# valeoai/NAF

Hardware: AMD Instinct MI355X
Metric: upsampled Mpixels/sec (NAF forward) (higher is better)
Workload: dtype bf16; 1 GPU; G1: 1x3x1024x1024 guidance, 1x768x64x64 features -> 1024x1024, window 7, per GPU; per_gpu_batch=1, global_batch=1, parallelism=batch-shard x1, scope=whole forward (conv stem + RoPE/pool + attention), weights=random-init NAF() defaults (dim 256, 4 heads), streams=2

## Files before the change

naf_amd/csrc/stem_conv1x1.hip:

```cpp
#include <type_traits>

#include "naf_common.h"

struct StemConv1Params {
    const bf16_t* x;
    bf16_t* y;
    const bf16_t* w;
    const float* bias;
    const float* gamma;
    const float* beta;
    const double* stats_in;
    double* stats_out;
    int32_t B, H, W;
    int32_t groups_per_image;
    int32_t groups_per_block;
    float eps;
    int64_t xs[3], ys[3];
    const void* img;
    const float* w0;
    const float* b0;
    int64_t ibs;
    int32_t is[4];
    bf16_t* kout;
    const float* tab_y;
    const float* tab_x;
    int64_t kst[3];
    int32_t cw;
    int32_t ncell;
    int32_t cells_per_block;
};

namespace {
constexpr int C1 = 128, WROW = C1 + 8, OROW1 = C1 + 8;
#ifndef NAF_C1X1_NW
#define NAF_C1X1_NW 4
#endif
#ifndef NAF_C1_ABL
#define NAF_C1_ABL 0
#endif
constexpr int NW1 = NAF_C1X1_NW;
typedef float f32x16_t __attribute__((ext_vector_type(16)));
constexpr float kLog2e = 1.4426950408889634f;
}

#ifdef NAF_C1_TIMING
__device__ unsigned long long g_c1_tim[4096 * 8];
#define C1_T(i) do { const unsigned long long now_ = __builtin_amdgcn_s_memtime(); tacc[i] += now_ - tlast; tlast = now_; } while (0)
#else
#define C1_T(i) do { } while (0)
#endif

template <bool IMG, typename T, bool DENSE, bool PLAIN = false, bool POOL = false>
__global__ __launch_bounds__(NW1 * 64, (NW1 <= 4 ? 2 : 1)) void stem_conv1x1_kernel(const StemConv1Params p) {
    static_assert(!(IMG && PLAIN), "the recomputed-conv0 input exists for the forward layer only");
    static_assert(!POOL || (DENSE && !IMG && !PLAIN), "key pooling: dense forward layer reading its input from memory");
#ifdef NAF_C1_TIMING
    unsigned long long tacc[8] = {0, 0, 0, 0, 0, 0, 0, 0}, tlast = __builtin_amdgcn_s_memtime();
#endif
    extern __shared__ __attribute__((aligned(16))) unsigned char smem[];
    bf16_t* wl = reinterpret_cast<bf16_t*>(smem);
    bf16_t* ot = wl + C1 * WROW;
    float* cvec = reinterpret_cast<float*>(ot + NW1 * 32 * OROW1);

    const int tid = threadIdx.x, lane = tid & 63;
    const int wave = __builtin_amdgcn_readfirstlane(tid >> 6);
    const int n32 = lane & 31, half = lane >> 5;
    const int b = blockIdx.y;

    const int gbase = POOL ? blockIdx.x * p.cells_per_block : blockIdx.x * p.groups_per_block;
    const int ngroups = POOL ? min(p.ncell, gbase + p.cells_per_block) : min(p.groups_per_image, gbase + p.groups_per_block);
    const int gstride = NW1;
    const int npx = p.H * p.W;
    bf16_t* otw = ot + wave * 32 * OROW1;

    const int chk = lane & 15, psub = lane >> 4;
    const bool xdense = DENSE || p.xs[1] == (int64_t)p.W * p.xs[2], ydense = DENSE || p.ys[1] == (int64_t)p.W * p.ys[2];
    const bf16_t* xbase = p.x + b * p.xs[0] + chk * 8;
    const uint32_t lane_x = (uint32_t)(psub * (int)p.xs[2] + chk * 8) * 2u, lane_y = (uint32_t)(psub * (int)p.ys[2] + chk * 8) * 2u;
    const int nfull = npx >> 5;
    auto pool_group_off = [&](int cell, int gi, const int64_t (&st)[3]) __attribute__((always_inline)) {
        const int cc = cell < ngroups ? cell : ngroups - 1;
        const int cy = cc / p.cw, cx = cc - cy * p.cw;
        return (int64_t)(cy * 16 + 2 * gi) * st[1] + (int64_t)cx * 16 * st[2];
    };
    auto load_group = [&](int g, u32x4_t (&raw)[8], int gi = 0) __attribute__((always_inline)) {
        if constexpr (POOL) {
            const char* xg = reinterpret_cast<const char*>(p.x + b * p.xs[0] + pool_group_off(g, gi, p.xs));
            uint32_t lx = lane_x;
            asm volatile("" : "+v"(lx));
#pragma unroll
            for (int it = 0; it < 8; ++it)
                raw[it] = *reinterpret_cast<const u32x4_t*>(xg + (uint32_t)(lx + (uint32_t)(((it >> 2) * (int)p.xs[1] + (it & 3) * 4 * (int)p.xs[2]) * 2)));
            return;
        }
        const int gc = g < ngroups ? g : ngroups - 1;
        if (DENSE || (xdense && gc < nfull)) {
            const char* xg = reinterpret_cast<const char*>(p.x + b * p.xs[0] + (int64_t)gc * 32 * p.xs[2]);
            uint32_t lx = lane_x;
            asm volatile("" : "+v"(lx));
#pragma unroll
            for (int it = 0; it < 8; ++it) raw[it] = *reinterpret_cast<const u32x4_t*>(xg + (uint32_t)(lx + (uint32_t)(it * 8 * (int)p.xs[2])));
            return;
        }
        if constexpr (!DENSE) {
#pragma unroll
        for (int it = 0; it < 8; ++it) {
            const int n = min(gc * 32 + it * 4 + psub, npx - 1);
            int64_t off;
            if (xdense) {
                off = (int64_t)n * p.xs[2];
            } else {
                const int yy = n / p.W, xx = n - yy * p.W;
                off = (int64_t)yy * p.xs[1] + (int64_t)xx * p.xs[2];
            }
            raw[it] = *reinterpret_cast<const u32x4_t*>(xbase + off);
        }
        }
    };
    constexpr int WCH = C1 * (C1 / 8), WIT = (WCH + NW1 * 64 - 1) / (NW1 * 64);
    u32x4_t wst[WIT];
#pragma unroll
    for (int i = 0; i < WIT; ++i) {
        const int ci = min(tid + i * NW1 * 64, WCH - 1);
        wst[i] = *reinterpret_cast<const u32x4_t*>(p.w + (ci >> 4) * C1 + (ci & 15) * 8);
    }
    u32x4_t raw[8];
    if constexpr (!IMG) load_group(gbase + wave, raw);
#pragma unroll
    for (int i = 0; i < WIT; ++i) {
        const int ci = tid + i * NW1 * 64;
        if (WCH % (NW1 * 64) == 0 || ci < WCH) *reinterpret_cast<u32x4_t*>(wl + (ci >> 4) * WROW + (ci & 15) * 8) = wst[i];
    }
    if (tid < C1) {
        const int c = tid, g = c >> 4;
        if constexpr (PLAIN) {
            cvec[c] = p.bias ? p.bias[c] : 0.f;
        } else {
            const double n = (double)p.H * (double)p.W * 16.0;
            double s1, s2;
            naf_gn_sums(p.stats_in, p.B, b, g, s1, s2);
            const double mean = s1 / n;
            double var = s2 / n - mean * mean;
            var = var > 0.0 ? var : 0.0;
            const float rstd = (float)(1.0 / sqrt(var + (double)p.eps));
            const float gmm = p.gamma[c];
            cvec[c] = p.bias[c];
            cvec[C1 + c] = gmm * rstd * kLog2e;
            cvec[2 * C1 + c] = (p.beta[c] - (float)mean * gmm * rstd) * kLog2e;
            if constexpr (IMG) cvec[3 * C1 + c] = p.b0[c];
        }
    }
    __syncthreads();

    float ga[8], gb[8];
#pragma unroll
    for (int e = 0; e < 8; ++e) {
        ga[e] = cvec[C1 + chk * 8 + e];
        gb[e] = cvec[2 * C1 + chk * 8 + e];
    }

    f32x2_t s1p[8], s2p[8];
#pragma unroll
    for (int g = 0; g < 8; ++g) s1p[g] = s2p[g] = f32x2_t{0.f, 0.f};

    float w0r[4][2];
    const T* ib = nullptr;
    if constexpr (IMG) {
        ib = reinterpret_cast<const T*>(p.img) + (int64_t)b * p.ibs;
#pragma unroll
        for (int m = 0; m < 4; ++m)
#pragma unroll
            for (int ks = 0; ks < 2; ++ks) {
                const int k = 2 * ks + half;
                w0r[m][ks] = (k < 3) ? p.w0[(32 * m + n32) * 3 + k] : 0.f;
            }
    }
    auto load_taps = [&](int g, float (&sv)[2]) __attribute__((always_inline)) {
        const int gc = g < ngroups ? g : ngroups - 1;
        const int n = min(gc * 32 + n32, npx - 1);
        const int yy = n / p.W, xx = n - yy * p.W;
        const int o = yy * p.is[2] + xx * p.is[3];
        sv[0] = (float)ib[o + half * p.is[1]];
        sv[1] = (float)ib[o + 2 * p.is[1]];
    };

    float sv[2] = {0.f, 0.f};
    int g = gbase + wave;
    int gi = 0;
    f32x4_t pacc[8];
    float ptab[16];
    bf16x8_t pax;
    const int pG = lane >> 4, pli = lane & 15;
    if constexpr (POOL) {
#pragma unroll
        for (int j = 0; j < 8; ++j) pacc[j] = f32x4_t{0.f, 0.f, 0.f, 0.f};
#pragma unroll
        for (int i = 0; i < 16; ++i) ptab[i] = 0.f;
#pragma unroll
        for (int i = 0; i < 8; ++i) pax[i] = (bf16_t)((8 * (pG & 1) + i == pli) ? 1.0f : 0.0f);
    }
    if constexpr (IMG) load_taps(g, sv);
    if constexpr (IMG) asm volatile("; conv1x1 first group landed" ::"v"(sv[0]), "v"(sv[1]));
    else asm volatile("; conv1x1 first group landed" ::"v"(raw[0]), "v"(raw[1]), "v"(raw[2]), "v"(raw[3]), "v"(raw[4]), "v"(raw[5]), "v"(raw[6]), "v"(raw[7]));
    C1_T(0);
    for (; g < ngroups; g += (POOL ? 0 : gstride)) {
        const int n0 = g * 32;
#ifdef NAF_C1_TIMING
        if constexpr (!IMG) {
            asm volatile("s_waitcnt vmcnt(8)" ::: "memory");
            C1_T(1);
        }
#endif
        const float* cv = cvec;

        f32x16_t acc[4];
#pragma unroll
        for (int m = 0; m < 4; ++m)
#pragma unroll
            for (int j = 0; j < 4; ++j) {
                const f32x4_t bj = *reinterpret_cast<const f32x4_t*>(cv + 32 * m + 8 * j + 4 * half);
#pragma unroll
                for (int i = 0; i < 4; ++i) acc[m][j * 4 + i] = bj[i];
            }
        if constexpr (IMG) {
#pragma unroll
            for (int mp = 0; mp < 2; ++mp) {
                f32x16_t a0[2];
#pragma unroll
                for (int q = 0; q < 2; ++q) {
#pragma unroll
                    for (int r = 0; r < 16; ++r) a0[q][r] = 0.f;
#pragma unroll
                    for (int ks = 0; ks < 2; ++ks) a0[q] = __builtin_amdgcn_mfma_f32_32x32x2f32(w0r[2 * mp + q][ks], sv[ks], a0[q], 0, 0, 0);
                }
#pragma unroll
                for (int q = 0; q < 2; ++q) {
                    const int m = 2 * mp + q;
#pragma unroll
                    for (int j = 0; j < 4; ++j) {
                        const int c0 = 32 * m + 8 * j + 4 * half;
                        const f32x4_t bj = *reinterpret_cast<const f32x4_t*>(cv + 3 * C1 + c0);
                        const f32x4_t gaj = *reinterpret_cast<const f32x4_t*>(cv + C1 + c0);
                        const f32x4_t gbj = *reinterpret_cast<const f32x4_t*>(cv + 2 * C1 + c0);
                        bf16x4_t o;
#pragma unroll
                        for (int e = 0; e < 2; ++e) {
                            const f32x2_t v = f32x2_t{a0[q][j * 4 + 2 * e], a0[q][j * 4 + 2 * e + 1]} + f32x2_t{bj[2 * e], bj[2 * e + 1]};
                            bf16x2_t xb;
                            xb[0] = (bf16_t)v[0];
                            xb[1] = (bf16_t)v[1];
                            const f32x2_t x = {(float)xb[0], (float)xb[1]};
                            const f32x2_t y = x * f32x2_t{gaj[2 * e], gaj[2 * e + 1]} + f32x2_t{gbj[2 * e], gbj[2 * e + 1]};
                            const f32x2_t u = f32x2_t{__builtin_amdgcn_exp2f(-y[0]), __builtin_amdgcn_exp2f(-y[1])} * kLog2e + kLog2e;
                            const f32x2_t r = y * f32x2_t{__builtin_amdgcn_rcpf(u[0]), __builtin_amdgcn_rcpf(u[1])};
                            o[2 * e] = (bf16_t)r[0];
                            o[2 * e + 1] = (bf16_t)r[1];
                        }
                        *reinterpret_cast<bf16x4_t*>(otw + n32 * OROW1 + c0) = o;
                    }
                }
            }
        } else {
#pragma unroll
        for (int it = 0; it < 8; ++it) {
            if constexpr (PLAIN || (NAF_C1_ABL & 1)) {
                *reinterpret_cast<u32x4_t*>(otw + (it * 4 + psub) * OROW1 + chk * 8) = raw[it];
                continue;
            }
            bf16x8_t o;
#pragma unroll
            for (int e = 0; e < 4; ++e) {
                const uint32_t w = raw[it][e];
                const f32x2_t x = {__uint_as_float(w << 16), __uint_as_float(w & 0xffff0000u)};
                const f32x2_t y = x * f32x2_t{ga[2 * e], ga[2 * e + 1]} + f32x2_t{gb[2 * e], gb[2 * e + 1]};
                const f32x2_t u = f32x2_t{__builtin_amdgcn_exp2f(-y[0]), __builtin_amdgcn_exp2f(-y[1])} * kLog2e + kLog2e;
                const f32x2_t r = y * f32x2_t{__builtin_amdgcn_rcpf(u[0]), __builtin_amdgcn_rcpf(u[1])};
                o[2 * e] = (bf16_t)r[0];
                o[2 * e + 1] = (bf16_t)r[1];
            }
            *reinterpret_cast<bf16x8_t*>(otw + (it * 4 + psub) * OROW1 + chk * 8) = o;
        }
        }
        C1_T(2);
        __builtin_amdgcn_sched_barrier(0);
        if constexpr (IMG) load_taps(g + gstride, sv);
        else if constexpr (POOL) {
            load_group(gi == 7 ? g + gstride : g, raw, (gi + 1) & 7);
            if (gi == 7) {
                const int cy = g / p.cw, cx = g - cy * p.cw;
                const float* ty = p.tab_y + (int64_t)(cy * 16 + 4 * pG) * 32 + pli;
                const float* tx = p.tab_x + (int64_t)(cx * 16 + 4 * pG) * 32 + pli;
#pragma unroll
                for (int i = 0; i < 4; ++i) {
                    ptab[i] = ty[i * 32];
                    ptab[4 + i] = ty[i * 32 + 16];
                    ptab[8 + i] = tx[i * 32];
                    ptab[12 + i] = tx[i * 32 + 16];
                }
            }
        }
        else if constexpr (!(NAF_C1_ABL & 16)) load_group(g + gstride, raw);
        __builtin_amdgcn_sched_barrier(0);
        {
            bf16x8_t bfr[2], war[2][4];
            auto frag = [&](int ks, int slot) __attribute__((always_inline)) {
                bfr[slot] = *reinterpret_cast<const bf16x8_t*>(otw + n32 * OROW1 + ks * 16 + half * 8);
#pragma unroll
                for (int m = 0; m < 4; ++m) war[slot][m] = *reinterpret_cast<const bf16x8_t*>(wl + (m * 32 + n32) * WROW + ks * 16 + half * 8);
            };
            frag(0, 0);
#pragma unroll
            for (int ks = 0; ks < 8; ++ks) {
                __builtin_amdgcn_sched_barrier(0);
                if (ks + 1 < 8) frag(ks + 1, (ks + 1) & 1);
                __builtin_amdgcn_sched_barrier(0);
#pragma unroll
                for (int m = 0; m < 4; ++m) {
                    if constexpr (!(NAF_C1_ABL & 2)) acc[m] = __builtin_amdgcn_mfma_f32_32x32x16_bf16(war[ks & 1][m], bfr[ks & 1], acc[m], 0, 0, 0);
                    else asm volatile("" ::"v"(war[ks & 1][m]), "v"(bfr[ks & 1]));
                }
            }
            __builtin_amdgcn_sched_barrier(0);
        }
#ifdef NAF_C1_TIMING
        asm volatile("" ::"v"(acc[0]), "v"(acc[1]), "v"(acc[2]), "v"(acc[3]));
        C1_T(3);
#endif
        const bool full = DENSE || g < nfull;
        auto epilogue = [&](auto fullc) __attribute__((always_inline)) {
            constexpr bool FULL = decltype(fullc)::value;
            const float vmask = (FULL || (n0 + n32) < npx) ? 1.0f : 0.0f;
#pragma unroll
            for (int m = 0; m < 4; ++m)
#pragma unroll
                for (int j = 0; j < 4; ++j) {
                    const f32x2_t v0 = f32x2_t{acc[m][j * 4], acc[m][j * 4 + 1]}, v1 = f32x2_t{acc[m][j * 4 + 2], acc[m][j * 4 + 3]};
                    bf16x4_t o;
                    o[0] = (bf16_t)v0[0]; o[1] = (bf16_t)v0[1]; o[2] = (bf16_t)v1[0]; o[3] = (bf16_t)v1[1];
                    const f32x2_t w0 = FULL ? v0 : v0 * vmask, w1 = FULL ? v1 : v1 * vmask;
                    if constexpr (!(NAF_C1_ABL & 4) && !POOL) {
                        s1p[m * 2 + (j >> 1)] += w0 + w1;
                        s2p[m * 2 + (j >> 1)] += w0 * w0 + w1 * w1;
                    }
                    *reinterpret_cast<bf16x4_t*>(otw + n32 * OROW1 + 32 * m + 8 * j + 4 * half) = o;
                }
            C1_T(4);
            bf16_t* yb = p.y + b * p.ys[0];
            if constexpr (POOL) {
                char* yg = reinterpret_cast<char*>(yb + pool_group_off(g, gi, p.ys));
                uint32_t ly = lane_y;
                asm volatile("" : "+v"(ly));
#pragma unroll
                for (int it = 0; it < 8; ++it) {
                    const u32x4_t v = *reinterpret_cast<const u32x4_t*>(otw + (it * 4 + psub) * OROW1 + chk * 8);
                    *reinterpret_cast<u32x4_t*>(yg + (uint32_t)(ly + (uint32_t)(((it >> 2) * (int)p.ys[1] + (it & 3) * 4 * (int)p.ys[2]) * 2))) = v;
                }
                return;
            }
            if (FULL && (DENSE || ydense)) {
                char* yg = reinterpret_cast<char*>(yb + (int64_t)g * 32 * p.ys[2]);
                uint32_t ly = lane_y;
                asm volatile("" : "+v"(ly));
#pragma unroll
                for (int it = 0; it < 8; ++it) {
                    const u32x4_t v = *reinterpret_cast<const u32x4_t*>(otw + (it * 4 + psub) * OROW1 + chk * 8);
                    if constexpr (!(NAF_C1_ABL & 8)) *reinterpret_cast<u32x4_t*>(yg + (int64_t)it * 8 * p.ys[2] + ly) = v;
                    else asm volatile("" ::"v"(v));
                }
                C1_T(5);
                return;
            }
            if constexpr (!(FULL && DENSE)) {
#pragma unroll
            for (int it = 0; it < 8; ++it) {
                const int pp = it * 4 + psub, ch = chk;
                const int n = n0 + pp;
                if (n < npx) {
                    int64_t off;
                    if (ydense) {
                        off = (int64_t)n * p.ys[2];
                    } else {
                        const int yy = n / p.W, xx = n - yy * p.W;
                        off = (int64_t)yy * p.ys[1] + (int64_t)xx * p.ys[2];
                    }
                    const u32x4_t v = *reinterpret_cast<const u32x4_t*>(otw + pp * OROW1 + ch * 8);
                    *reinterpret_cast<u32x4_t*>(yb + off + ch * 8) = v;
                }
            }
            }
        };
        if constexpr (DENSE) {
            epilogue(std::true_type{});
        } else {
            if (full) epilogue(std::true_type{});
            else epilogue(std::false_type{});
        }
        if constexpr (POOL) {
            bf16x8_t pay;
            {
                const bf16_t one = (bf16_t)(((2 * gi + (pG >> 1)) == pli) ? 1.0f : 0.0f);
#pragma unroll
                for (int i = 0; i < 8; ++i) pay[i] = one;
            }
            const bf16_t* tb = otw + (8 * pG + (pli >> 2)) * OROW1 + (pli & 3) * 4;
#pragma unroll
            for (int j = 0; j < 8; ++j) {
                const bf16x4_t lo = __builtin_amdgcn_ds_read_tr16_b64_v4bf16((NAF_LDS bf16x4_t*)(tb + 16 * j));
                const bf16x4_t hi = __builtin_amdgcn_ds_read_tr16_b64_v4bf16((NAF_LDS bf16x4_t*)(tb + 4 * OROW1 + 16 * j));
                const bf16x8_t bt = {lo[0], lo[1], lo[2], lo[3], hi[0], hi[1], hi[2], hi[3]};
                pacc[j] = __builtin_amdgcn_mfma_f32_16x16x32_bf16((j & 1) ? pax : pay, bt, pacc[j], 0, 0, 0);
            }
            if (gi == 7) {
                const int cy = g / p.cw, cx = g - cy * p.cw;
                bf16_t* kc = p.kout + b * p.kst[0] + (int64_t)cy * p.kst[1] + (int64_t)cx * p.kst[2];
#pragma unroll
                for (int hh = 0; hh < 2; ++hh) {
                    float o[4] = {0.f, 0.f, 0.f, 0.f};
#pragma unroll
                    for (int i = 0; i < 4; ++i) {
                        float r1, r2;
                        naf_rope_rotate(pacc[4 * hh][i], pacc[4 * hh + 2][i], ptab[i], ptab[4 + i], r1, r2);
                        o[0] += r1;
                        o[2] += r2;
                        naf_rope_rotate(pacc[4 * hh + 1][i], pacc[4 * hh + 3][i], ptab[8 + i], ptab[12 + i], r1, r2);
                        o[1] += r1;
                        o[3] += r2;
                    }
#pragma unroll
                    for (int q = 0; q < 4; ++q) {
                        o[q] += __shfl_xor(o[q], 16);
                        o[q] += __shfl_xor(o[q], 32);
                    }
                    const float v = pG == 0 ? o[0] : pG == 1 ? o[1] : pG == 2 ? o[2] : o[3];
                    kc[64 * hh + lane] = (bf16_t)(v * (1.0f / 256.0f));
                }
#pragma unroll
                for (int j = 0; j < 8; ++j) pacc[j] = f32x4_t{0.f, 0.f, 0.f, 0.f};
                gi = 0;
                g += gstride;
            } else {
                ++gi;
            }
        }
    }

    if constexpr (IMG) asm volatile("; conv1x1 loop drained" ::"v"(sv[0]), "v"(sv[1]));
    else asm volatile("; conv1x1 loop drained" ::"v"(raw[0]), "v"(raw[1]), "v"(raw[2]), "v"(raw[3]), "v"(raw[4]), "v"(raw[5]), "v"(raw[6]), "v"(raw[7]));
#ifdef NAF_C1_TIMING
    if (lane == 0 && blockIdx.x < 512)
        for (int i = 0; i < 8; ++i) g_c1_tim[(blockIdx.x * NW1 + wave) * 8 + i] = tacc[i];
#endif
    if (p.stats_out) {
        __syncthreads();
        float* red = reinterpret_cast<float*>(ot);
#pragma unroll
        for (int gq = 0; gq < 8; ++gq) {
            float a = s1p[gq][0] + s1p[gq][1], q = s2p[gq][0] + s2p[gq][1];
#pragma unroll
            for (int o = 32; o > 0; o >>= 1) {
                a += __shfl_xor(a, o);
                q += __shfl_xor(q, o);
            }
            if (lane == 0) {
                red[wave * 16 + gq] = a;
                red[wave * 16 + 8 + gq] = q;
            }
        }
        __syncthreads();
        if (tid < 16) {
            float a = 0.f;
#pragma unroll
            for (int wv = 0; wv < NW1; ++wv) a += red[wv * 16 + tid];
            atomicAdd(&naf_gn_slot(p.stats_out, p.B, b, blockIdx.x)[(tid & 7) * 2 + (tid >> 3)], (double)a);
        }
    }
}

int naf_stem_conv1x1_keys_ok(const naf_stem_conv_args* a, const naf_key_pool_args* kp) {
    return a->ksize == 1 && a->first == nullptr && a->stats_in != nullptr && a->stats_out == nullptr && (a->channels == 0 || a->channels == 128) &&
           a->H == 16 * kp->h && a->W == 16 * kp->w && a->x_stride[1] == (int64_t)a->W * a->x_stride[2] &&
           a->y_stride[1] == (int64_t)a->W * a->y_stride[2] && a->x_stride[1] * 2 < 0x7fffffffLL && a->y_stride[1] * 2 < 0x7fffffffLL;
}

int naf_launch_stem_conv1x1(const naf_stem_conv_args* a, hipStream_t s, const naf_key_pool_args* kp) {
    StemConv1Params p;
    p.x = static_cast<const bf16_t*>(a->x);
    p.y = static_cast<bf16_t*>(a->y);
    p.w = static_cast<const bf16_t*>(a->w_packed);
    p.bias = a->bias; p.gamma = a->gn_weight; p.beta = a->gn_bias;
    p.stats_in = a->stats_in; p.stats_out = a->stats_out;
    p.B = a->B; p.H = a->H; p.W = a->W; p.eps = a->eps;
    for (int i = 0; i < 3; ++i) { p.xs[i] = a->x_stride[i]; p.ys[i] = a->y_stride[i]; }
    p.groups_per_image = (int)(((int64_t)a->H * a->W + 31) / 32);
    const size_t lds = (size_t)(C1 * WROW + NW1 * 32 * OROW1) * 2 + 4 * C1 * sizeof(float);
    const int64_t slots = (int64_t)naf_cu_count() * (NW1 <= 4 ? 2 : 1) * NW1;
    const int64_t total = (int64_t)p.groups_per_image * a->B;
    const int64_t gpw = (total + slots - 1) / slots;
    static const int gpw_knob = [] { const char* e = naf_knob("NAF_C1X1_GPW"); return e ? atoi(e) : 0; }();
    const int64_t gpw_eff = gpw_knob > 0 ? gpw_knob : gpw;
    p.groups_per_block = (int32_t)(gpw_eff * NW1);
    int64_t nbx = (p.groups_per_image + p.groups_per_block - 1) / p.groups_per_block;
    if (nbx < 1) nbx = 1;
    if (a->B > 65535) {
        naf_set_error("naf_stem_conv_fwd: batch %d out of range", a->B);
        return NAF_ERR_INVALID;
    }
    p.img = nullptr; p.w0 = nullptr; p.b0 = nullptr; p.ibs = 0;
    for (int i = 0; i < 4; ++i) p.is[i] = 0;
    p.kout = nullptr; p.tab_y = p.tab_x = nullptr; p.cw = p.ncell = p.cells_per_block = 0;
    for (int i = 0; i < 3; ++i) p.kst[i] = 0;
    if (kp != nullptr) {
        if (!naf_stem_conv1x1_keys_ok(a, kp)) {
            naf_set_error("naf_stem_conv_keys_fwd: the 1x1 kernel needs 16 x 16 pixel cells, dense rows, stats_out == NULL and first == NULL");
            return NAF_ERR_UNSUPPORTED;
        }
        p.kout = static_cast<bf16_t*>(kp->k_lr); p.tab_y = kp->tab_y; p.tab_x = kp->tab_x;
        for (int i = 0; i < 3; ++i) p.kst[i] = kp->k_stride[i];
        p.cw = kp->w; p.ncell = kp->h * kp->w;
        const int64_t cpw = ((int64_t)p.ncell * a->B + slots - 1) / slots;
        p.cells_per_block = (int32_t)(cpw * NW1);
        nbx = (p.ncell + p.cells_per_block - 1) / p.cells_per_block;
    }
    int variant = 0;
    if (a->first != nullptr) {
        const naf_stem_conv0_args* f = a->first;
        const int64_t span = 2 * llabs(f->image_stride[1]) + (int64_t)(a->H - 1) * llabs(f->image_stride[2]) +
                             (int64_t)(a->W - 1) * llabs(f->image_stride[3]);
        if (span >= 0x7fffffffLL) {
            naf_set_error("naf_stem_conv_fwd: first: image too large for 32-bit tap offsets (span %lld elements)", (long long)span);
            return NAF_ERR_UNSUPPORTED;
        }
        p.img = f->image; p.w0 = f->weight; p.b0 = f->bias; p.ibs = f->image_stride[0];
        for (int i = 0; i < 4; ++i) p.is[i] = (int32_t)f->image_stride[i];
        variant = f->image_dtype == NAF_BF16 ? 2 : 1;
    }
    const dim3 grid((uint32_t)nbx, (uint32_t)a->B), blk(NW1 * 64);
    if (kp != nullptr) {
        auto kern = stem_conv1x1_kernel<false, float, true, false, true>;
        if (hipFuncSetAttribute(reinterpret_cast<const void*>(kern), hipFuncAttributeMaxDynamicSharedMemorySize, (int)lds) != hipSuccess) {
            naf_set_error("naf_stem_conv_keys_fwd: cannot reserve %zu bytes of LDS", (size_t)lds);
            return NAF_ERR_LAUNCH;
        }
        hipLaunchKernelGGL(kern, grid, blk, lds, s, p);
        return naf_check_launch("stem_conv1x1_kernel<keys>");
    }
#define NAF_LAUNCH_1X1(KERN)                                                                                              \
    do {                                                                                                                  \
        if (hipFuncSetAttribute(reinterpret_cast<const void*>(KERN), hipFuncAttributeMaxDynamicSharedMemorySize, (int)lds) != hipSuccess) { \
            naf_set_error("naf_stem_conv_fwd: cannot reserve %zu bytes of LDS", (size_t)lds);                             \
            return NAF_ERR_LAUNCH;                                                                                        \
        }                                                                                                                 \
        hipLaunchKernelGGL(KERN, grid, blk, lds, s, p);                                                                   \
    } while (0)
    const bool dense = (a->x_stride[1] == (int64_t)a->W * a->x_stride[2] || a->first != nullptr) &&
                       a->y_stride[1] == (int64_t)a->W * a->y_stride[2] && (((int64_t)a->H * a->W) % 32 == 0);
    if (a->stats_in == nullptr) {
        if (dense) NAF_LAUNCH_1X1((stem_conv1x1_kernel<false, float, true, true>));
        else NAF_LAUNCH_1X1((stem_conv1x1_kernel<false, float, false, true>));
    } else if (dense) {
        if (variant == 0) NAF_LAUNCH_1X1((stem_conv1x1_kernel<false, float, true>));
        else if (variant == 1) NAF_LAUNCH_1X1((stem_conv1x1_kernel<true, float, true>));
        else NAF_LAUNCH_1X1((stem_conv1x1_kernel<true, bf16_t, true>));
    } else {
        if (variant == 0) NAF_LAUNCH_1X1((stem_conv1x1_kernel<false, float, false>));
        else if (variant == 1) NAF_LAUNCH_1X1((stem_conv1x1_kernel<true, float, false>));
        else NAF_LAUNCH_1X1((stem_conv1x1_kernel<true, bf16_t, false>));
    }
#undef NAF_LAUNCH_1X1
    return naf_check_launch("stem_conv1x1_kernel");
}
```

Before: 566.8 Mpix/s.

## Keep conv1x1 weights resident in AGPRs and switch to 16x16x32 MFMA

Loads the 128x128 weight matrix once into accumulation registers (AGPRs) per lane, staging it through the per-wave tile region so the dedicated weight LDS area can be dropped. The GEMM moves from 32x32x16 MFMAs with per-step weight fragment LDS reads to 16x16x32 MFMAs using inline asm. The work is split into two 16-pixel halves, so the epilogue and store of one half can interleave with the compute of the next. Pool table loads are moved next to their use, and non-dense inputs are now loaded inside the loop rather than prefetched. This removes LDS weight traffic and shrinks the LDS footprint, at the cost of many AGPRs, hand-placed nops for hazards, and less overlap of the next group's load in the non-dense path.

```diff
diff --git a/naf_amd/csrc/stem_conv1x1.hip b/naf_amd/csrc/stem_conv1x1.hip
--- a/naf_amd/csrc/stem_conv1x1.hip
+++ b/naf_amd/csrc/stem_conv1x1.hip
@@ -31,7 +31,7 @@
 };
 
 namespace {
-constexpr int C1 = 128, WROW = C1 + 8, OROW1 = C1 + 8;
+constexpr int C1 = 128, OROW1 = C1 + 8;
 #ifndef NAF_C1X1_NW
 #define NAF_C1X1_NW 4
 #endif
@@ -58,13 +58,15 @@
     unsigned long long tacc[8] = {0, 0, 0, 0, 0, 0, 0, 0}, tlast = __builtin_amdgcn_s_memtime();
 #endif
     extern __shared__ __attribute__((aligned(16))) unsigned char smem[];
-    bf16_t* wl = reinterpret_cast<bf16_t*>(smem);
-    bf16_t* ot = wl + C1 * WROW;
+    bf16_t* ot = reinterpret_cast<bf16_t*>(smem);
     float* cvec = reinterpret_cast<float*>(ot + NW1 * 32 * OROW1);
 
     const int tid = threadIdx.x, lane = tid & 63;
     const int wave = __builtin_amdgcn_readfirstlane(tid >> 6);
     const int n32 = lane & 31, half = lane >> 5;
+    const int c16 = lane & 15, kgrp = lane >> 4;
+    const int pix = (c16 >= 4 && c16 < 12) ? 2 * (c16 - 4) : (c16 < 4 ? 2 * c16 + 1 : 2 * c16 - 15);
+    const int kq = ((kgrp & 1) << 1) | (kgrp >> 1);
     const int b = blockIdx.y;
 
     const int gbase = POOL ? blockIdx.x * p.cells_per_block : blockIdx.x * p.groups_per_block;
@@ -117,7 +119,8 @@
         }
         }
     };
-    constexpr int WCH = C1 * (C1 / 8), WIT = (WCH + NW1 * 64 - 1) / (NW1 * 64);
+    constexpr int WROW = OROW1, WCH = C1 * (C1 / 8), WIT = (WCH + NW1 * 64 - 1) / (NW1 * 64);
+    static_assert(C1 * WROW <= NW1 * 32 * OROW1, "the weights are staged through the waves' tile region");
     u32x4_t wst[WIT];
 #pragma unroll
     for (int i = 0; i < WIT; ++i) {
@@ -125,11 +128,11 @@
         wst[i] = *reinterpret_cast<const u32x4_t*>(p.w + (ci >> 4) * C1 + (ci & 15) * 8);
     }
     u32x4_t raw[8];
-    if constexpr (!IMG) load_group(gbase + wave, raw);
+    if constexpr (!IMG && DENSE) load_group(gbase + wave, raw);
 #pragma unroll
     for (int i = 0; i < WIT; ++i) {
         const int ci = tid + i * NW1 * 64;
-        if (WCH % (NW1 * 64) == 0 || ci < WCH) *reinterpret_cast<u32x4_t*>(wl + (ci >> 4) * WROW + (ci & 15) * 8) = wst[i];
+        if (WCH % (NW1 * 64) == 0 || ci < WCH) *reinterpret_cast<u32x4_t*>(ot + (ci >> 4) * WROW + (ci & 15) * 8) = wst[i];
     }
     if (tid < C1) {
         const int c = tid, g = c >> 4;
@@ -151,17 +154,31 @@
         }
     }
     __syncthreads();
+    bf16x8_t wreg[32];
+    {
+        const bf16_t* wp = ot + c16 * WROW + kq * 8;
+#pragma unroll
+        for (int t = 0; t < 8; ++t)
+#pragma unroll
+            for (int ks = 0; ks < 4; ++ks) wreg[t * 4 + ks] = *reinterpret_cast<const bf16x8_t*>(wp + t * 16 * WROW + ks * 32);
+    }
+#pragma unroll
+    for (int i = 0; i < 32; i += 8)
+        asm volatile("; conv1x1 weights landed" ::"a"(wreg[i]), "a"(wreg[i + 1]), "a"(wreg[i + 2]), "a"(wreg[i + 3]), "a"(wreg[i + 4]), "a"(wreg[i + 5]), "a"(wreg[i + 6]), "a"(wreg[i + 7]));
+    __syncthreads();
 
     float ga[8], gb[8];
-#pragma unroll
-    for (int e = 0; e < 8; ++e) {
-        ga[e] = cvec[C1 + chk * 8 + e];
-        gb[e] = cvec[2 * C1 + chk * 8 + e];
-    }
-
-    f32x2_t s1p[8], s2p[8];
-#pragma unroll
-    for (int g = 0; g < 8; ++g) s1p[g] = s2p[g] = f32x2_t{0.f, 0.f};
+    auto load_gn = [&]() __attribute__((always_inline)) {
+#pragma unroll
+        for (int e = 0; e < 8; ++e) {
+            ga[e] = cvec[C1 + chk * 8 + e];
+            gb[e] = cvec[2 * C1 + chk * 8 + e];
+        }
+    };
+
+    float s1[8], s2[8];
+#pragma unroll
+    for (int g = 0; g < 8; ++g) s1[g] = s2[g] = 0.f;
 
     float w0r[4][2];
     const T* ib = nullptr;
@@ -188,20 +205,14 @@
     int g = gbase + wave;
     int gi = 0;
     f32x4_t pacc[8];
-    float ptab[16];
-    bf16x8_t pax;
     const int pG = lane >> 4, pli = lane & 15;
     if constexpr (POOL) {
 #pragma unroll
         for (int j = 0; j < 8; ++j) pacc[j] = f32x4_t{0.f, 0.f, 0.f, 0.f};
-#pragma unroll
-        for (int i = 0; i < 16; ++i) ptab[i] = 0.f;
-#pragma unroll
-        for (int i = 0; i < 8; ++i) pax[i] = (bf16_t)((8 * (pG & 1) + i == pli) ? 1.0f : 0.0f);
     }
     if constexpr (IMG) load_taps(g, sv);
     if constexpr (IMG) asm volatile("; conv1x1 first group landed" ::"v"(sv[0]), "v"(sv[1]));
-    else asm volatile("; conv1x1 first group landed" ::"v"(raw[0]), "v"(raw[1]), "v"(raw[2]), "v"(raw[3]), "v"(raw[4]), "v"(raw[5]), "v"(raw[6]), "v"(raw[7]));
+    else if constexpr (DENSE) asm volatile("; conv1x1 first group landed" ::"v"(raw[0]), "v"(raw[1]), "v"(raw[2]), "v"(raw[3]), "v"(raw[4]), "v"(raw[5]), "v"(raw[6]), "v"(raw[7]));
     C1_T(0);
     for (; g < ngroups; g += (POOL ? 0 : gstride)) {
         const int n0 = g * 32;
@@ -212,16 +223,8 @@
         }
 #endif
         const float* cv = cvec;
-
-        f32x16_t acc[4];
-#pragma unroll
-        for (int m = 0; m < 4; ++m)
-#pragma unroll
-            for (int j = 0; j < 4; ++j) {
-                const f32x4_t bj = *reinterpret_cast<const f32x4_t*>(cv + 32 * m + 8 * j + 4 * half);
-#pragma unroll
-                for (int i = 0; i < 4; ++i) acc[m][j * 4 + i] = bj[i];
-            }
+        if constexpr (!DENSE && !IMG) load_group(g, raw);
+        if constexpr (!IMG && !PLAIN && !(NAF_C1_ABL & 1)) load_gn();
         if constexpr (IMG) {
 #pragma unroll
             for (int mp = 0; mp < 2; ++mp) {
@@ -286,74 +289,51 @@
         if constexpr (IMG) load_taps(g + gstride, sv);
         else if constexpr (POOL) {
             load_group(gi == 7 ? g + gstride : g, raw, (gi + 1) & 7);
-            if (gi == 7) {
-                const int cy = g / p.cw, cx = g - cy * p.cw;
-                const float* ty = p.tab_y + (int64_t)(cy * 16 + 4 * pG) * 32 + pli;
-                const float* tx = p.tab_x + (int64_t)(cx * 16 + 4 * pG) * 32 + pli;
-#pragma unroll
-                for (int i = 0; i < 4; ++i) {
-                    ptab[i] = ty[i * 32];
-                    ptab[4 + i] = ty[i * 32 + 16];
-                    ptab[8 + i] = tx[i * 32];
-                    ptab[12 + i] = tx[i * 32 + 16];
-                }
-            }
-        }
-        else if constexpr (!(NAF_C1_ABL & 16)) load_group(g + gstride, raw);
+        }
+        else if constexpr (DENSE && !(NAF_C1_ABL & 16)) load_group(g + gstride, raw);
         __builtin_amdgcn_sched_barrier(0);
-        {
-            bf16x8_t bfr[2], war[2][4];
-            auto frag = [&](int ks, int slot) __attribute__((always_inline)) {
-                bfr[slot] = *reinterpret_cast<const bf16x8_t*>(otw + n32 * OROW1 + ks * 16 + half * 8);
-#pragma unroll
-                for (int m = 0; m < 4; ++m) war[slot][m] = *reinterpret_cast<const bf16x8_t*>(wl + (m * 32 + n32) * WROW + ks * 16 + half * 8);
-            };
-            frag(0, 0);
-#pragma unroll
-            for (int ks = 0; ks < 8; ++ks) {
-                __builtin_amdgcn_sched_barrier(0);
-                if (ks + 1 < 8) frag(ks + 1, (ks + 1) & 1);
-                __builtin_amdgcn_sched_barrier(0);
-#pragma unroll
-                for (int m = 0; m < 4; ++m) {
-                    if constexpr (!(NAF_C1_ABL & 2)) acc[m] = __builtin_amdgcn_mfma_f32_32x32x16_bf16(war[ks & 1][m], bfr[ks & 1], acc[m], 0, 0, 0);
-                    else asm volatile("" ::"v"(war[ks & 1][m]), "v"(bfr[ks & 1]));
-                }
-            }
-            __builtin_amdgcn_sched_barrier(0);
-        }
-#ifdef NAF_C1_TIMING
-        asm volatile("" ::"v"(acc[0]), "v"(acc[1]), "v"(acc[2]), "v"(acc[3]));
-        C1_T(3);
-#endif
+        f32x4_t acc[8];
+        bf16x8_t bfr[2];
+        const bf16_t* bsrc = otw + pix * OROW1 + kq * 8;
+        const float* bsrcv = cv + 4 * kgrp;
+        auto bias_init = [&]() __attribute__((always_inline)) {
+#pragma unroll
+            for (int t = 0; t < 8; ++t) acc[t] = *reinterpret_cast<const f32x4_t*>(bsrcv + 16 * t);
+        };
         const bool full = DENSE || g < nfull;
-        auto epilogue = [&](auto fullc) __attribute__((always_inline)) {
+        bf16_t* yb = p.y + b * p.ys[0];
+        auto epilogue = [&](auto fullc, int h) __attribute__((always_inline)) {
             constexpr bool FULL = decltype(fullc)::value;
-            const float vmask = (FULL || (n0 + n32) < npx) ? 1.0f : 0.0f;
-#pragma unroll
-            for (int m = 0; m < 4; ++m)
-#pragma unroll
-                for (int j = 0; j < 4; ++j) {
-                    const f32x2_t v0 = f32x2_t{acc[m][j * 4], acc[m][j * 4 + 1]}, v1 = f32x2_t{acc[m][j * 4 + 2], acc[m][j * 4 + 3]};
-                    bf16x4_t o;
-                    o[0] = (bf16_t)v0[0]; o[1] = (bf16_t)v0[1]; o[2] = (bf16_t)v1[0]; o[3] = (bf16_t)v1[1];
-                    const f32x2_t w0 = FULL ? v0 : v0 * vmask, w1 = FULL ? v1 : v1 * vmask;
-                    if constexpr (!(NAF_C1_ABL & 4) && !POOL) {
-                        s1p[m * 2 + (j >> 1)] += w0 + w1;
-                        s2p[m * 2 + (j >> 1)] += w0 * w0 + w1 * w1;
-                    }
-                    *reinterpret_cast<bf16x4_t*>(otw + n32 * OROW1 + 32 * m + 8 * j + 4 * half) = o;
-                }
+            const float vmask = (FULL || (n0 + 16 * h + pix) < npx) ? 1.0f : 0.0f;
+#pragma unroll
+            for (int t = 0; t < 8; ++t) {
+                const f32x2_t v0 = f32x2_t{acc[t][0], acc[t][1]}, v1 = f32x2_t{acc[t][2], acc[t][3]};
+                bf16x4_t o;
+                o[0] = (bf16_t)v0[0]; o[1] = (bf16_t)v0[1]; o[2] = (bf16_t)v1[0]; o[3] = (bf16_t)v1[1];
+                const f32x2_t w0 = FULL ? v0 : v0 * vmask, w1 = FULL ? v1 : v1 * vmask;
+                if constexpr (!(NAF_C1_ABL & 4) && !POOL) {
+                    const f32x2_t a2 = w0 + w1, q2 = w0 * w0 + w1 * w1;
+                    s1[t] += a2[0] + a2[1];
+                    s2[t] += q2[0] + q2[1];
+                }
+                *reinterpret_cast<bf16x4_t*>(otw + (16 * h + pix) * OROW1 + 16 * t + 4 * kgrp) = o;
+            }
             C1_T(4);
-            bf16_t* yb = p.y + b * p.ys[0];
+        };
+        auto store_half = [&](auto fullc, int h) __attribute__((always_inline)) {
+            constexpr bool FULL = decltype(fullc)::value;
             if constexpr (POOL) {
                 char* yg = reinterpret_cast<char*>(yb + pool_group_off(g, gi, p.ys));
                 uint32_t ly = lane_y;
                 asm volatile("" : "+v"(ly));
-#pragma unroll
-                for (int it = 0; it < 8; ++it) {
-                    const u32x4_t v = *reinterpret_cast<const u32x4_t*>(otw + (it * 4 + psub) * OROW1 + chk * 8);
-                    *reinterpret_cast<u32x4_t*>(yg + (uint32_t)(ly + (uint32_t)(((it >> 2) * (int)p.ys[1] + (it & 3) * 4 * (int)p.ys[2]) * 2))) = v;
+                u32x4_t v[4];
+#pragma unroll
+                for (int i = 0; i < 4; ++i) v[i] = *reinterpret_cast<const u32x4_t*>(otw + ((4 * h + i) * 4 + psub) * OROW1 + chk * 8);
+                __builtin_amdgcn_sched_barrier(0);
+#pragma unroll
+                for (int i = 0; i < 4; ++i) {
+                    const int it = 4 * h + i;
+                    *reinterpret_cast<u32x4_t*>(yg + (uint32_t)(ly + (uint32_t)(((it >> 2) * (int)p.ys[1] + (it & 3) * 4 * (int)p.ys[2]) * 2))) = v[i];
                 }
                 return;
             }
@@ -361,19 +341,24 @@
                 char* yg = reinterpret_cast<char*>(yb + (int64_t)g * 32 * p.ys[2]);
                 uint32_t ly = lane_y;
                 asm volatile("" : "+v"(ly));
-#pragma unroll
-                for (int it = 0; it < 8; ++it) {
-                    const u32x4_t v = *reinterpret_cast<const u32x4_t*>(otw + (it * 4 + psub) * OROW1 + chk * 8);
-                    if constexpr (!(NAF_C1_ABL & 8)) *reinterpret_cast<u32x4_t*>(yg + (int64_t)it * 8 * p.ys[2] + ly) = v;
-                    else asm volatile("" ::"v"(v));
+                u32x4_t v[4];
+#pragma unroll
+                for (int i = 0; i < 4; ++i) v[i] = *reinterpret_cast<const u32x4_t*>(otw + ((4 * h + i) * 4 + psub) * OROW1 + chk * 8);
+                __builtin_amdgcn_sched_barrier(0);
+#pragma unroll
+                for (int i = 0; i < 4; ++i) {
+                    if constexpr (!(NAF_C1_ABL & 8)) *reinterpret_cast<u32x4_t*>(yg + (int64_t)(4 * h + i) * 8 * p.ys[2] + ly) = v[i];
+                    else asm volatile("" ::"v"(v[i]));
                 }
                 C1_T(5);
                 return;
             }
             if constexpr (!(FULL && DENSE)) {
-#pragma unroll
-            for (int it = 0; it < 8; ++it) {
-                const int pp = it * 4 + psub, ch = chk;
+            int ps_ = psub, ch_ = chk;
+            asm volatile("" : "+v"(ps_), "+v"(ch_));
+#pragma unroll
+            for (int it = 4 * h; it < 4 * h + 4; ++it) {
+                const int pp = it * 4 + ps_, ch = ch_;
                 const int n = n0 + pp;
                 if (n < npx) {
                     int64_t off;
@@ -389,14 +374,50 @@
             }
             }
         };
-        if constexpr (DENSE) {
-            epilogue(std::true_type{});
-        } else {
-            if (full) epilogue(std::true_type{});
-            else epilogue(std::false_type{});
+        bias_init();
+        bfr[0] = *reinterpret_cast<const bf16x8_t*>(bsrc);
+#pragma unroll
+        for (int h = 0; h < 2; ++h) {
+#pragma unroll
+            for (int ks = 0; ks < 4; ++ks) {
+                __builtin_amdgcn_sched_barrier(0);
+                if (ks + 1 < 4) bfr[(ks + 1) & 1] = *reinterpret_cast<const bf16x8_t*>(bsrc + 16 * h * OROW1 + (ks + 1) * 32);
+                else if (h == 0) bfr[0] = *reinterpret_cast<const bf16x8_t*>(bsrc + 16 * OROW1);
+                __builtin_amdgcn_sched_barrier(0);
+#pragma unroll
+                for (int t = 0; t < 8; ++t) {
+                    if (t == 0) asm volatile("s_nop 1");
+                    if constexpr (!(NAF_C1_ABL & 2))
+                        asm volatile("v_mfma_f32_16x16x32_bf16 %0, %1, %2, %0" : "+v"(acc[t]) : "a"(wreg[t * 4 + ks]), "v"(bfr[ks & 1]));
+                    else asm volatile("" : "+v"(acc[t]) : "a"(wreg[t * 4 + ks]), "v"(bfr[ks & 1]));
+                }
+            }
+            __builtin_amdgcn_sched_barrier(0);
+            if constexpr (!(NAF_C1_ABL & 2)) asm volatile("s_nop 15" : "+v"(acc[0]), "+v"(acc[1]), "+v"(acc[2]), "+v"(acc[3]), "+v"(acc[4]), "+v"(acc[5]), "+v"(acc[6]), "+v"(acc[7]));
+            __builtin_amdgcn_sched_barrier(0);
+            C1_T(3);
+            if constexpr (DENSE) {
+                epilogue(std::true_type{}, h);
+            } else {
+                if (full) epilogue(std::true_type{}, h);
+                else epilogue(std::false_type{}, h);
+            }
+            if constexpr (DENSE) {
+                store_half(std::true_type{}, h);
+            } else {
+                if (full) store_half(std::true_type{}, h);
+                else store_half(std::false_type{}, h);
+            }
+            if (h == 0) bias_init();
         }
         if constexpr (POOL) {
-            bf16x8_t pay;
+            bf16x8_t pax, pay;
+            {
+                int pl_ = pli;
+                asm volatile("" : "+v"(pl_));
+#pragma unroll
+                for (int i = 0; i < 8; ++i) pax[i] = (bf16_t)((8 * (pG & 1) + i == pl_) ? 1.0f : 0.0f);
+            }
             {
                 const bf16_t one = (bf16_t)(((2 * gi + (pG >> 1)) == pli) ? 1.0f : 0.0f);
 #pragma unroll
@@ -412,6 +433,18 @@
             }
             if (gi == 7) {
                 const int cy = g / p.cw, cx = g - cy * p.cw;
+                float ptab[16];
+                {
+                    const float* ty = p.tab_y + (int64_t)(cy * 16 + 4 * pG) * 32 + pli;
+                    const float* tx = p.tab_x + (int64_t)(cx * 16 + 4 * pG) * 32 + pli;
+#pragma unroll
+                    for (int i = 0; i < 4; ++i) {
+                        ptab[i] = ty[i * 32];
+                        ptab[4 + i] = ty[i * 32 + 16];
+                        ptab[8 + i] = tx[i * 32];
+                        ptab[12 + i] = tx[i * 32 + 16];
+                    }
+                }
                 bf16_t* kc = p.kout + b * p.kst[0] + (int64_t)cy * p.kst[1] + (int64_t)cx * p.kst[2];
 #pragma unroll
                 for (int hh = 0; hh < 2; ++hh) {
@@ -445,7 +478,7 @@
     }
 
     if constexpr (IMG) asm volatile("; conv1x1 loop drained" ::"v"(sv[0]), "v"(sv[1]));
-    else asm volatile("; conv1x1 loop drained" ::"v"(raw[0]), "v"(raw[1]), "v"(raw[2]), "v"(raw[3]), "v"(raw[4]), "v"(raw[5]), "v"(raw[6]), "v"(raw[7]));
+    else if constexpr (DENSE) asm volatile("; conv1x1 loop drained" ::"v"(raw[0]), "v"(raw[1]), "v"(raw[2]), "v"(raw[3]), "v"(raw[4]), "v"(raw[5]), "v"(raw[6]), "v"(raw[7]));
 #ifdef NAF_C1_TIMING
     if (lane == 0 && blockIdx.x < 512)
         for (int i = 0; i < 8; ++i) g_c1_tim[(blockIdx.x * NW1 + wave) * 8 + i] = tacc[i];
@@ -455,7 +488,7 @@
         float* red = reinterpret_cast<float*>(ot);
 #pragma unroll
         for (int gq = 0; gq < 8; ++gq) {
-            float a = s1p[gq][0] + s1p[gq][1], q = s2p[gq][0] + s2p[gq][1];
+            float a = s1[gq], q = s2[gq];
 #pragma unroll
             for (int o = 32; o > 0; o >>= 1) {
                 a += __shfl_xor(a, o);
@@ -492,7 +525,7 @@
     p.B = a->B; p.H = a->H; p.W = a->W; p.eps = a->eps;
     for (int i = 0; i < 3; ++i) { p.xs[i] = a->x_stride[i]; p.ys[i] = a->y_stride[i]; }
     p.groups_per_image = (int)(((int64_t)a->H * a->W + 31) / 32);
-    const size_t lds = (size_t)(C1 * WROW + NW1 * 32 * OROW1) * 2 + 4 * C1 * sizeof(float);
+    const size_t lds = (size_t)(NW1 * 32 * OROW1) * 2 + 4 * C1 * sizeof(float);
     const int64_t slots = (int64_t)naf_cu_count() * (NW1 <= 4 ? 2 : 1) * NW1;
     const int64_t total = (int64_t)p.groups_per_image * a->B;
     const int64_t gpw = (total + slots - 1) / slots;
```

Result: no change. 569.0 Mpix/s, median of 6 (+0.4%).
